# AlexandreRouma/SDRPlusPlus

Hardware: NVIDIA H100
Metric: complex IQ MSamples/s through FFT + 8-VFO WFM chain (higher is better)
Workload: dtype f32

## Files before the change

### sdrplusplus_b200/csrc/api.cpp

```cpp
#include "../../include/b200dsp.h"
#include "engine.h"
#include <chrono>
#include <map>
#include <cmath>
#include <cstdio>
#include <cstring>
#include <cstdlib>
#include <algorithm>

using namespace b200;

static int g_device = -1;

static int ensure_device() {
    int n = 0;
    cudaError_t e = cudaGetDeviceCount(&n);
    if (e != cudaSuccess || n <= 0) {
        set_error("no usable CUDA device (%s): libb200dsp has no CPU fallback", e == cudaSuccess ? "0 devices" : cudaGetErrorString(e));
        cudaGetLastError();
        return B200_ENODEV;
    }
    if (g_device < 0) { g_device = 0; }
    B200_CK(cudaSetDevice(g_device));
    return 0;
// ... 59 lines not shown
    out->mode = pl.mode;
    out->predec_ratio = pl.predec_ratio;
    out->interp = pl.interp;
    out->decim = pl.decim;
    out->ntaps = (int)pl.rtaps.size();
    out->taps_per_phase = pl.taps_per_phase;
    if (pl.use_decim) {
        const DecimPlan* dp = find_decim_plan(pl.predec_ratio);
        if (!dp) { set_error("no decimation plan for ratio %d", pl.predec_ratio); return B200_ENOPLAN; }
        out->nstages = (int)dp->stages.size();
        for (int i = 0; i < out->nstages && i < 8; i++) {
            out->stage_decim[i] = dp->stages[i].decim;
            out->stage_taps[i] = (int)dp->stages[i].taps.size();
        }
    }
    return 0;
}

static int bytes_per_sample(int fmt) { return fmt == B200_FMT_CF32 ? 8 : (fmt == B200_FMT_CS16 ? 4 : 2); }
static int ilog2(int n) { int l = 0; while ((1 << l) < n) { l++; } return l; }

struct FftCore {
    FftPlanDev plan;
    DevBuf tw, twf, win, work;
    int size = 0, nz = 0, window = 0;
    int create(int size_, int nz_, int window_, int max_batch = 1) {
        if (size_ < 8 || size_ > (1 << 22) || (size_ & (size_ - 1))) { set_error("FFT size %d must be a power of two in [8, 4194304]", size_); return B200_EINVAL; }
        if (nz_ < 1 || nz_ > size_) { set_error("bad nz %d", nz_); return B200_EINVAL; }
        size = size_; nz = nz_; window = window_;
        memset(&plan, 0, sizeof(plan));
        plan.N = size; plan.logN = ilog2(size);
        if (size <= 8192) { plan.N1 = size; plan.logN1 = plan.logN; plan.N2 = 1; plan.logN2 = 0; }
        else {
            plan.logN1 = (plan.logN + 1) / 2; plan.N1 = 1 << plan.logN1;
            plan.logN2 = plan.logN - plan.logN1; plan.N2 = 1 << plan.logN2;
        }
        plan.TW = std::max(plan.N1, plan.N2); plan.logTW = ilog2(plan.TW);
        std::vector<float2> t((size_t)plan.TW);
        for (int k = 0; k < plan.TW; k++) {
            double a = -2.0 * 3.14159265358979323846 * (double)k / (double)plan.TW;
            t[k] = make_float2((float)std::cos(a), (float)std::sin(a));
        }
        int rc;
        if ((rc = tw.alloc(t.size() * sizeof(float2)))) { return rc; }
        B200_CK(cudaMemcpy(tw.p, t.data(), t.size() * sizeof(float2), cudaMemcpyHostToDevice));
        std::vector<float> w = fft_window(window, nz);
        if ((rc = win.alloc((size_t)nz * sizeof(float)))) { return rc; }
        B200_CK(cudaMemcpy(win.p, w.data(), (size_t)nz * sizeof(float), cudaMemcpyHostToDevice));
        if ((rc = work.alloc((size_t)size * sizeof(float2) * (size_t)(max_batch > 0 ? max_batch : 1)))) { return rc; }
        plan.tw = tw.as<float2>(); plan.window = win.as<float>(); plan.nz = nz;
        plan.tw_fine = nullptr;
        if (plan.N2 > 1) {
            const int nf = size / plan.TW;
            std::vector<float2> f((size_t)nf);
            for (int j = 0; j < nf; j++) {
                double a = -2.0 * 3.14159265358979323846 * (double)j / (double)size;
                f[j] = make_float2((float)std::cos(a), (float)std::sin(a));
            }
            if ((rc = twf.alloc(f.size() * sizeof(float2)))) { return rc; }
            B200_CK(cudaMemcpy(twf.p, f.data(), f.size() * sizeof(float2), cudaMemcpyHostToDevice));
            plan.tw_fine = twf.as<float2>();
        }
        B200_CK(cudaDeviceSynchronize());
        return 0;
    }
};

static_assert(sizeof(b200_rds_symbol) == 8 && sizeof(RdsSym) == sizeof(b200_rds_symbol), "one RDS symbol record is 8 bytes");
struct RdsCore {
    DevBuf state, taps, bank;
    RdsState init;
    RdsJob proto;
    int create(cudaStream_t s);
    int reset(cudaStream_t s);
    RdsJob job(const float2* in, int n, RdsSym* out, int out_cap, int* count) const {
        RdsJob J = proto;
        J.in = in; J.n = n; J.out = out; J.out_cap = out_cap; J.count = count;
        return J;
    }
};
int RdsCore::create(cudaStream_t s) {
    const std::vector<float> bp = bandpass_c_taps(0.0, 2375.0, 100.0, 5000.0, false);
    const std::vector<float> bk = mm_interp_bank(RDS_MM_PHASES, RDS_MM_TAPS);
    const int nt = (int)bp.size() / 2;
// ... 49 lines not shown

struct b200_fe {
    double fs = 0;
    int max_chunk = 0;
    Scheduler sch;
    cudaStream_t own_stream = nullptr, copy_stream = nullptr, fft_stream = nullptr, tail_stream = nullptr, join_stream = nullptr;
    cudaEvent_t ev_tail_done[FE_SLOTS] = {};
    cudaEvent_t ev_fft_go = nullptr, ev_fft_done = nullptr, ev_lines_free = nullptr;
    bool overlap = true;
    bool lines_busy = false;
    float* lines_override = nullptr;
    bool fft_async = true;
    bool fft_join_pending = false;
    std::vector<std::unique_ptr<VfoSlot>> vfos;
    std::mutex mtx;
    DevBuf in_dev[FE_SLOTS];
    bool fft_on = false;
    FftCore fft;
    double fft_rate = 0;
    int skip = 0;
    DevBuf frame, lines;
    int max_lines = 0;
    unsigned long long pos = 0, fstart = 0;
    cudaEvent_t ev_h2d[FE_SLOTS] = {}, ev_compute[FE_SLOTS] = {}, ev_out[FE_SLOTS] = {};
    bool slot_used[FE_SLOTS] = {};
    int max_inflight = 2;
    unsigned long long nsub = 0, nwait = 0;
    int fft_serial = 0;
    int host_direct = -1;
    long long host_ns[4] = { 0, 0, 0, 0 };
    float scale16 = 1.0f / 32768.0f, scale8 = 1.0f / 128.0f;
    int decim = 1;
    double fs_eff = 0;
    bool dc_block = false, invert_iq = false;
    Chain pre;
    Scheduler sch_pre;
    DevBuf pp[FE_SLOTS];
    DevBuf dc_state, dc_segA, dc_segB;
    int max_eff = 0;
    int* rds_count = nullptr;
    struct RdsPend { int id, n_in, bound; };
    std::vector<RdsPend> rds_pend[FE_SLOTS];
    b200_outputs* rds_out[FE_SLOTS] = {};
};

static float fe_ingest_scale(const b200_fe* fe, int fmt) {
// ... 297 lines not shown
    if (!strcmp(key, "s1_stages")) { kernels_set_xd_tma_stages(value); return 0; }
    if (!strcmp(key, "s1_diag")) { kernels_set_xd_tma_diag(value); return 0; }
    if (!strcmp(key, "s1_ctas")) { kernels_set_xd_tma_ctas(value); return 0; }
    if (!strcmp(key, "tails") || !strncmp(key, "ft_", 3)) {
        if (b200_fe_vfo_count(fe) > 0) { set_error("'%s' must be chosen before VFOs are added", key); return B200_ESTATE; }
        if (!strcmp(key, "tails")) { kernels_set_tail_variant(value >= 1 ? 1 : 0); fe->sch.fuse.on = value >= 2; return 0; }
        if (!strcmp(key, "ft_ob")) { fe->sch.fuse.ob_force = value; return 0; }
        if (!strcmp(key, "ft_obmax")) { fe->sch.fuse.ob_max = value; return 0; }
        if (!strcmp(key, "ft_smem_kb")) { fe->sch.fuse.smem_limit = value * 1024; return 0; }
        if (!strcmp(key, "ft_threads")) { fe->sch.fuse.threads = value; return 0; }
        if (!strcmp(key, "ft_direct")) { fe->sch.fuse.direct = value != 0; return 0; }
        if (!strcmp(key, "ft_prereg")) { fe->sch.fuse.pre_reg = value; return 0; }
        if (!strcmp(key, "ft_regall")) { fe->sch.fuse.reg_all = value != 0; return 0; }
    }
    if (!strcmp(key, "fft")) { kernels_set_fft_variant(value); return 0; }
    if (!strcmp(key, "fft_cta")) { kernels_set_fft_cta(value); return 0; }
    if (!strcmp(key, "host_direct")) { fe->host_direct = value; return 0; }
    if (!strcmp(key, "inflight")) {
        if (value < 1 || value > FE_SLOTS) { set_error("inflight: 1 ... %d", FE_SLOTS); return B200_EINVAL; }
        fe->max_inflight = value;
        return 0;
    }
    if (!strcmp(key, "fft_serial")) { fe->fft_serial = value; return 0; }
    if (!strcmp(key, "graph")) { fe->sch.graph_tails = value; if (value == 0) { fe->sch.drop_graphs(); } return 0; }
    if (!strcmp(key, "graph_max_count")) { fe->sch.graph_max_count = value; return 0; }
    if (!strcmp(key, "pdl")) { kernels_set_pdl(value); fe->sch.drop_graphs(); return 0; }
    if (!strcmp(key, "tail_split")) { fe->sch.tail_split = value; fe->sch.drop_graphs(); return 0; }
    if (!strcmp(key, "time_s1")) { fe->sch.time_s1 = value != 0; for (auto& t : fe->sch.timers) { t.used = 0; } return 0; }
    set_error("unknown option %s", key);
    return B200_EINVAL;
}

extern "C" int b200_fe_s1_stats(b200_fe* fe, double* ms_total, int* launches) {
    if (!fe || !ms_total || !launches) { set_error("null argument"); return B200_EINVAL; }
    return fe->sch.s1_stats(ms_total, launches);
}
extern "C" int b200_fe_group_stats(b200_fe* fe, int group, double* ms_total, int* launches) {
    if (!fe || !ms_total || !launches) { set_error("null argument"); return B200_EINVAL; }
    return fe->sch.group_stats(group, ms_total, launches);
}

extern "C" int b200_fe_reset(b200_fe* fe) {
    if (!fe) { set_error("null fe"); return B200_EINVAL; }
    std::lock_guard<std::mutex> lck(fe->mtx);
    B200_CK(cudaDeviceSynchronize());
    for (auto& v : fe->vfos) {
// ... 49 lines not shown
    const unsigned long long pos = fe->pos, end = pos + (unsigned long long)count;
    const unsigned long long nz = (unsigned long long)fe->fft.nz, interval = nz + (unsigned long long)fe->skip;
    const int bps = bytes_per_sample(fmt);
    const float isc = fe_ingest_scale(fe, fmt);
    fe->fft.plan.in_scale = isc;
    cudaStream_t main_s = fe->sch.stream;
    const bool async = fe->fft_async || fe->sch.tail_stream != nullptr;
    float* const lines_base = fe->lines_override ? fe->lines_override : fe->lines.as<float>();
    cudaStream_t s = async ? fe->fft_stream : main_s;
    bool forked = false;
    cudaEvent_t t_fft = nullptr;
    auto fork = [&]() -> int {
        if (async && !forked) {
            B200_CK(cudaEventRecord(fe->ev_fft_go, main_s));
            B200_CK(cudaStreamWaitEvent(s, fe->ev_fft_go, 0));
            if (fe->lines_busy) { B200_CK(cudaStreamWaitEvent(s, fe->ev_lines_free, 0)); }
            trace_mark("fft start", s);
            t_fft = fe->sch.timer_begin(2, s);
            forked = true;
        }
        return 0;
    };
    int rc = 0;
    if (fe->fstart < pos) {
        const unsigned long long fend = fe->fstart + nz;
        const unsigned long long lo = pos, hi = std::min(fend, end);
        if (hi > lo) {
            if ((rc = fork())) { return rc; }
            cudaError_t e = launch_convert_cf32(dptr, fmt, fe->frame.as<float2>() + (size_t)(lo - fe->fstart), (int)(hi - lo), isc, s);
            if (e != cudaSuccess) { return cuda_fail(e, "launch_convert_cf32"); }
            fe->sch.launches++;
        }
        if (fend <= end) {
            if ((rc = fork())) { return rc; }
            int nl = 0;
            cudaError_t e = launch_fft_frame(fe->fft.plan, fe->frame.p, FMT_CF32, fe->fft.work.as<float2>(), lines_base, nullptr, s, &nl);
            if (e != cudaSuccess) { return cuda_fail(e, "launch_fft_frame"); }
            fe->sch.launches += nl;
            (*nlines)++;
            fe->fstart += interval;
        }
    }
    if (fe->fstart >= pos && fe->fstart + nz <= end) {
        int nb = (int)((end - fe->fstart - nz) / interval) + 1;
        if (*nlines + nb > fe->max_lines) { set_error("FFT line buffer overflow"); return B200_ECAP; }
        if ((rc = fork())) { return rc; }
        const char* src = (const char*)dptr + (size_t)(fe->fstart - pos) * bps;
        int nl = 0;
        cudaError_t e = launch_fft_frames(fe->fft.plan, src, fmt, fe->fft.work.as<float2>(),
                                          lines_base + (size_t)(*nlines) * fe->fft.size, nullptr, s, &nl, nb,
                                          (long long)interval * bps);
        if (e != cudaSuccess) { return cuda_fail(e, "launch_fft_frames"); }
        fe->sch.launches += nl;
        *nlines += nb;
        fe->fstart += interval * (unsigned long long)nb;
    }
    if (fe->fstart < end && fe->fstart >= pos) {
        const unsigned long long lo = fe->fstart, hi = end;
        if (hi > lo) {
            if ((rc = fork())) { return rc; }
            const char* src = (const char*)dptr + (size_t)(lo - pos) * bps;
            cudaError_t e = launch_convert_cf32(src, fmt, fe->frame.as<float2>(), (int)(hi - lo), isc, s);
            if (e != cudaSuccess) { return cuda_fail(e, "launch_convert_cf32"); }
            fe->sch.launches++;
        }
    }
    if (forked) {
        if (t_fft) { B200_CK(cudaEventRecord(t_fft, s)); }
        trace_mark("fft done", s);
        B200_CK(cudaEventRecord(fe->ev_fft_done, s));
        fe->fft_join_pending = true;
        if (fe->fft_serial && s != main_s) { B200_CK(cudaStreamWaitEvent(main_s, fe->ev_fft_done, 0)); }
    }
    fe->pos = end;
    return 0;
}

extern "C" int b200_fe_submit(b200_fe* fe, const void* iq, int count, int in_fmt, int in_mem, b200_outputs* out) {
    if (!fe || !out || (count > 0 && !iq)) { set_error("null argument"); return B200_EINVAL; }
    if (count < 0 || count > fe->max_chunk) { set_error("count %d exceeds max_chunk %d", count, fe->max_chunk); return B200_ECAP; }
    if (in_fmt < 0 || in_fmt > 2) { set_error("bad input format"); return B200_EINVAL; }
    if (fe->nsub - fe->nwait >= (unsigned long long)fe->max_inflight) { set_error("%d chunks already in flight: call b200_fe_wait", fe->max_inflight); return B200_ESTATE; }
    std::lock_guard<std::mutex> lck(fe->mtx);
    const long long hp0 = host_clock_ns();
    apply_pending(fe);
    const int slot = (int)(fe->nsub % FE_SLOTS);
    cudaStream_t s = fe->sch.stream;
// ... 958 lines not shown
```

### sdrplusplus_b200/csrc/fft_reg.cuh

```cuda
#pragma once

__device__ constexpr float FR_COS[16] = { 1.000000000e+00f, 9.807852804e-01f, 9.238795325e-01f, 8.314696123e-01f, 7.071067812e-01f, 5.555702330e-01f,
                                          3.826834324e-01f, 1.950903220e-01f, 0.0f, -1.950903220e-01f, -3.826834324e-01f, -5.555702330e-01f,
                                          -7.071067812e-01f, -8.314696123e-01f, -9.238795325e-01f, -9.807852804e-01f };
__device__ constexpr float FR_SIN[16] = { 0.000000000e+00f, 1.950903220e-01f, 3.826834324e-01f, 5.555702330e-01f, 7.071067812e-01f, 8.314696123e-01f,
                                          9.238795325e-01f, 9.807852804e-01f, 1.0f, 9.807852804e-01f, 9.238795325e-01f, 8.314696123e-01f,
                                          7.071067812e-01f, 5.555702330e-01f, 3.826834324e-01f, 1.950903220e-01f };

template <int R, int K>
__device__ __forceinline__ float2 fr_mul_w(float2 v) {
    constexpr int k32 = K * (32 / R);
    if constexpr (k32 == 0) { return v; }
    else if constexpr (k32 == 8) { return make_float2(v.y, -v.x); }
    else if constexpr (k32 == 4) { return make_float2((v.x + v.y) * RSQRT2, (v.y - v.x) * RSQRT2); }
    else if constexpr (k32 == 12) { return make_float2((v.y - v.x) * RSQRT2, -(v.x + v.y) * RSQRT2); }
    else {
        constexpr float c = FR_COS[k32], s = FR_SIN[k32];
        return make_float2(fmaf(v.y, s, v.x * c), fmaf(-v.x, s, v.y * c));
    }
}
template <int R, int H, int I>
__device__ __forceinline__ void fr_stage(float2 (&a)[R]) {
    constexpr int blk = I / H, j = I % H, i0 = blk * 2 * H + j;
    const float2 u = a[i0], v = a[i0 + H];
    a[i0] = make_float2(u.x + v.x, u.y + v.y);
    a[i0 + H] = fr_mul_w<2 * H, j>(make_float2(u.x - v.x, u.y - v.y));
    if constexpr (I + 1 < R / 2) { fr_stage<R, H, I + 1>(a); }
    else if constexpr (H > 1) { fr_stage<R, H / 2, 0>(a); }
}
template <int R>
__device__ __forceinline__ void fr_dft(float2 (&a)[R]) { fr_stage<R, R / 2, 0>(a); }
template <int R>
__host__ __device__ constexpr int fr_brev(int c) {
    int r = 0;
    for (int bit = 1; bit < R; bit <<= 1) { r = (r << 1) | ((c & bit) ? 1 : 0); }
    return r;
}
template <int RA, int RB> struct FrGeom {
    static constexpr int n = RA * RB;
    static constexpr int TP = RA > RB ? RA : RB;
    static constexpr int crow = RB + 1;
    static constexpr int pitch = ((RA * crow + 13) / 16) * 16 + 2;
};

template <int RA, int RB>
__device__ __forceinline__ void fr_transform(float2 (&v)[RA > RB ? RA : RB], float2* ex, int t, const float2* __restrict__ tw, int twsh) {
    using G = FrGeom<RA, RB>;
    if (t < RB) {
        float2 a[RA];
#pragma unroll
        for (int i = 0; i < RA; i++) { a[i] = v[i]; }
        fr_dft<RA>(a);
#pragma unroll
        for (int c = 0; c < RA; c++) {
            float2 y = a[fr_brev<RA>(c)];
            if (c > 0) { y = cmulf(y, __ldg(tw + ((size_t)(t * c) << twsh))); }
            ex[c * G::crow + t] = y;
        }
    }
    __syncthreads();
    if (t < RA) {
        float2 b[RB];
#pragma unroll
        for (int i = 0; i < RB; i++) { b[i] = ex[t * G::crow + i]; }
        fr_dft<RB>(b);
#pragma unroll
        for (int i = 0; i < RB; i++) { v[i] = b[i]; }
    }
}

template <int FMT, int RA, int RB, int C, int MINB>
__global__ void __launch_bounds__(C * FrGeom<RA, RB>::TP, MINB) k_fftr_p1(const __grid_constant__ FftPlanDev pl, const void* __restrict__ src0,
                                                                    float2* __restrict__ work0, long long src_stride_bytes) {
    using G = FrGeom<RA, RB>;
    extern __shared__ __align__(16) float2 smem[];
    const int N2 = pl.N2;
    const void* src = reinterpret_cast<const char*>(src0) + (size_t)blockIdx.y * src_stride_bytes;
    float2* work = work0 + (size_t)blockIdx.y * pl.N;
    const int col = threadIdx.x % C, t = threadIdx.x / C;
    const int n2 = blockIdx.x * C + col;
    float2 v[G::TP];
    if (t < RB) {
#pragma unroll
        for (int a = 0; a < RA; a++) { v[a] = load_windowed<FMT>(pl, src, (a * RB + t) * N2 + n2); }
    }
    fr_transform<RA, RB>(v, smem + col * G::pitch, t, pl.tw, pl.logTW - pl.logN1);
    if (t < RA) {
        const int s = pl.logN - pl.logTW;
        const unsigned msk = (1u << s) - 1u;
#pragma unroll
        for (int d = 0; d < RB; d++) {
            const int k1 = t + RA * d;
            const unsigned e = (unsigned)k1 * (unsigned)n2;
            const float2 w = cmulf(__ldg(pl.tw + (e >> s)), __ldg(pl.tw_fine + (e & msk)));
            work[(size_t)k1 * N2 + n2] = cmulf(v[fr_brev<RB>(d)], w);
        }
    }
}

template <int RA, int RB, int R>
__global__ void __launch_bounds__(R * FrGeom<RA, RB>::TP) k_fftr_p2(const __grid_constant__ FftPlanDev pl, const float2* __restrict__ work0,
                                                                    float* __restrict__ out_db0) {
    using G = FrGeom<RA, RB>;
    extern __shared__ __align__(16) float2 smem[];
    const int N1 = pl.N1, N2 = pl.N2;
    const float2* work = work0 + (size_t)blockIdx.y * pl.N;
    float* out_db = out_db0 + (size_t)blockIdx.y * pl.N;
    const int t = threadIdx.x % G::TP, row = threadIdx.x / G::TP;
    const int r0 = blockIdx.x * R;
    float2 v[G::TP];
    if (t < RB) {
        const float2* __restrict__ p = work + (size_t)(r0 + row) * N2 + t;
#pragma unroll
        for (int a = 0; a < RA; a++) { v[a] = __ldg(p + a * RB); }
    }
    fr_transform<RA, RB>(v, smem + row * G::pitch, t, pl.tw, pl.logTW - pl.logN2);
    __syncthreads();
    float* T = reinterpret_cast<float*>(smem);
    const float nf = 1.0f / ((float)pl.N * (float)pl.N);
    if (t < RA) {
#pragma unroll
        for (int d = 0; d < RB; d++) { T[(t + RA * d) * (R + 1) + row] = power_db(v[fr_brev<RB>(d)], nf); }
    }
    __syncthreads();
    for (int idx = threadIdx.x; idx < G::n * R; idx += R * G::TP) {
        const int k2 = idx / R, rl = idx - k2 * R;
        out_db[(size_t)(r0 + rl) + (size_t)N1 * k2] = T[k2 * (R + 1) + rl];
    }
}
```

### sdrplusplus_b200/csrc/kernels.cu

```cuda
#include "kernels.cuh"
#include <unordered_map>
#include <mutex>
#include <math.h>
#include <string.h>
#include <algorithm>

template <int FMT>
__device__ __forceinline__ float2 load_iq(const void* __restrict__ p, long long i, float sc) {
    if (FMT == FMT_CF32) {
        return __ldg(reinterpret_cast<const float2*>(p) + i);
    }
    else if (FMT == FMT_CS16) {
        short2 v = __ldg(reinterpret_cast<const short2*>(p) + i);
        return make_float2((float)v.x * sc, (float)v.y * sc);
    }
    else {
        char2 v = __ldg(reinterpret_cast<const char2*>(p) + i);
        return make_float2((float)v.x * sc, (float)v.y * sc);
    }
}

template <int FMT>
__device__ __forceinline__ float2 load_x(const XdParams& p, long long i) {
    if (i >= 0) {
// ... 435 lines not shown
        for (int t = tid; t < per * C; t += nthr) {
            int c, bi;
            if (BATCH_INNER) { c = t & (C - 1); bi = t >> logC; }
            else { bi = t & (per - 1); c = t >> logper; }
            const int base = bi * 2;
            float2 a0 = s[fft_addr<BATCH_INNER>(base + 0, c, C, pitch)];
            float2 a1 = s[fft_addr<BATCH_INNER>(base + 1, c, C, pitch)];
            s[fft_addr<BATCH_INNER>(base + 0, c, C, pitch)] = cadd(a0, a1);
            s[fft_addr<BATCH_INNER>(base + 1, c, C, pitch)] = csub(a0, a1);
        }
        __syncthreads();
    }
}

__device__ __forceinline__ int bitrev(int k, int bits) { return (int)(__brev((unsigned)k) >> (32 - bits)); }

__device__ __forceinline__ float power_db(float2 X, float normFactSq) {
    float m2 = (X.x * X.x + X.y * X.y) * normFactSq;
    float l = log2f(m2);
    if (isinf(l)) { l = copysignf(127.0f, l); }
    return l * 3.01029995663981209120f;
}

template <int FMT>
__device__ __forceinline__ float2 load_windowed(const FftPlanDev& pl, const void* __restrict__ src, int n) {
    if (n >= pl.nz) { return make_float2(0.0f, 0.0f); }
    float2 x = load_iq<FMT>(src, n, pl.in_scale);
    float w = __ldg(pl.window + n);
    return make_float2(x.x * w, x.y * w);
}

template <int FMT>
__global__ void __launch_bounds__(512) k_fft_single(const __grid_constant__ FftPlanDev pl, const void* __restrict__ src0,
                                                      float* __restrict__ out_db0, float2* __restrict__ out_raw,
                                                      long long src_stride_bytes) {
    extern __shared__ __align__(16) float2 smem[];
    const int N = pl.N;
    const void* src = reinterpret_cast<const char*>(src0) + (size_t)blockIdx.y * src_stride_bytes;
    float* out_db = out_db0 + (size_t)blockIdx.y * N;
#pragma unroll 4
    for (int i = threadIdx.x; i < N; i += blockDim.x) { smem[padf(i)] = load_windowed<FMT>(pl, src, i); }
    __syncthreads();
    fft_dif_smem<false>(smem, pl.logN, 1, N, pl.tw, pl.logTW);
    const float nf = 1.0f / ((float)N * (float)N);
    for (int k = threadIdx.x; k < N; k += blockDim.x) {
        float2 X = smem[padf(bitrev(k, pl.logN))];
        out_db[k] = power_db(X, nf);
        if (out_raw) { out_raw[k] = X; }
    }
}

template <int FMT>
__global__ void __launch_bounds__(512) k_fft_p1(const __grid_constant__ FftPlanDev pl, const void* __restrict__ src0,
                                                  float2* __restrict__ work0, int C, long long src_stride_bytes) {
    extern __shared__ __align__(16) float2 smem[];
    const int N1 = pl.N1, N2 = pl.N2;
    const void* src = reinterpret_cast<const char*>(src0) + (size_t)blockIdx.y * src_stride_bytes;
    float2* work = work0 + (size_t)blockIdx.y * pl.N;
    const int c0 = blockIdx.x * C;
#pragma unroll 4
    for (int t = threadIdx.x; t < N1 * C; t += blockDim.x) {
        int n1 = t / C, c = t - n1 * C;
        smem[padf(t)] = load_windowed<FMT>(pl, src, n1 * N2 + c0 + c);
    }
    __syncthreads();
    fft_dif_smem<true>(smem, pl.logN1, C, 0, pl.tw, pl.logTW);
    const float scale = -2.0f / (float)pl.N;
    for (int t = threadIdx.x; t < N1 * C; t += blockDim.x) {
        int k1 = t / C, c = t - k1 * C;
        float2 a = smem[padf(bitrev(k1, pl.logN1) * C + c)];
        int n2 = c0 + c;
        float sn, cs;
        sincospif((float)(k1 * n2) * scale, &sn, &cs);
        work[(size_t)k1 * N2 + n2] = cmulf(a, make_float2(cs, sn));
    }
}

__global__ void __launch_bounds__(512) k_fft_p2(const __grid_constant__ FftPlanDev pl, const float2* __restrict__ work0,
                                                  float* __restrict__ out_db0, float2* __restrict__ out_raw, int R) {
    extern __shared__ __align__(16) float2 smem[];
    const int N1 = pl.N1, N2 = pl.N2;
    const float2* work = work0 + (size_t)blockIdx.y * pl.N;
    float* out_db = out_db0 + (size_t)blockIdx.y * pl.N;
    const int pitch = N2 + 1;
    const int r0 = blockIdx.x * R;
#pragma unroll 4
// ... 536 lines not shown
cudaError_t launch_m2s(const M2SParams& p, cudaStream_t s) {
    if (p.max_n <= 0 || p.njobs <= 0) { return cudaSuccess; }
    dim3 grid(cdiv(p.max_n, 256), p.njobs);
    k_m2s<<<grid, 256, 0, s>>>(p);
    return cudaGetLastError();
}
cudaError_t launch_rxl(const RxlParams& p, cudaStream_t s) {
    if (p.max_n <= 0 || p.njobs <= 0) { return cudaSuccess; }
    dim3 grid(cdiv(p.max_n, 256), p.njobs);
    k_rxl<<<grid, 256, 0, s>>>(p);
    return cudaGetLastError();
}
cudaError_t launch_scale(const ScaleParams& p, cudaStream_t s) {
    if (p.max_n <= 0 || p.njobs <= 0) { return cudaSuccess; }
    dim3 grid(cdiv(p.max_n, 256), p.njobs);
    k_scale<<<grid, 256, 0, s>>>(p);
    return cudaGetLastError();
}
cudaError_t launch_carry(const CarryParams& p, cudaStream_t s) {
    if (p.njobs <= 0) { return cudaSuccess; }
    return launch_chain(k_carry, dim3((unsigned)p.njobs), dim3(256), 0, s, p);
}

template <int FMT>
static cudaError_t launch_fft_fmt(const FftPlanDev& pl, const void* src, float2* work, float* out_db, float2* out_raw,
                                  cudaStream_t s, int* nlaunch, int nbatch, long long src_stride_bytes) {
    cudaError_t e;
    if (pl.N1 == pl.N) {
        size_t smem = ((size_t)pl.N + (pl.N >> 4) + 2) * sizeof(float2);
        e = set_smem(k_fft_single<FMT>, smem);
        if (e != cudaSuccess) { return e; }
        int thr = pl.N / 8 < 32 ? 32 : (pl.N / 8 > 512 ? 512 : pl.N / 8);
        k_fft_single<FMT><<<dim3(1, nbatch), thr, smem, s>>>(pl, src, out_db, out_raw, src_stride_bytes);
        if (nlaunch) { (*nlaunch)++; }
        return cudaGetLastError();
    }
    if (g_fft_variant >= 1 && !out_raw && pl.tw_fine && pl.logN1 >= 8 && pl.logN1 <= 10 && pl.logN2 >= 8 && pl.logN2 <= 10) {
#define FR_P1(RA, RB, CC)                                                                                      \
        do {                                                                                                   \
            const size_t sm = (size_t)CC * FrGeom<RA, RB>::pitch * sizeof(float2);                             \
            e = set_smem(k_fftr_p1<FMT, RA, RB, CC, 2>, sm);                                                   \
            if (e != cudaSuccess) { return e; }                                                                \
            k_fftr_p1<FMT, RA, RB, CC, 2><<<dim3(pl.N2 / CC, nbatch), CC * FrGeom<RA, RB>::TP, sm, s>>>(pl, src, work, src_stride_bytes); \
        } while (0)
#define FR_P2(RA, RB, RR)                                                                                      \
        do {                                                                                                   \
            const size_t sm = (size_t)RR * FrGeom<RA, RB>::pitch * sizeof(float2);                             \
            e = set_smem(k_fftr_p2<RA, RB, RR>, sm);                                                           \
            if (e != cudaSuccess) { return e; }                                                                \
            k_fftr_p2<RA, RB, RR><<<dim3(pl.N1 / RR, nbatch), RR * FrGeom<RA, RB>::TP, sm, s>>>(pl, work, out_db); \
        } while (0)
        if (g_fft_cta == 4) {
            if (pl.logN1 == 10) { FR_P1(32, 32, 4); } else if (pl.logN1 == 9) { FR_P1(16, 32, 4); } else { FR_P1(16, 16, 4); }
        }
        else {
            if (pl.logN1 == 10) { FR_P1(32, 32, 8); } else if (pl.logN1 == 9) { FR_P1(16, 32, 8); } else { FR_P1(16, 16, 8); }
        }
        e = cudaGetLastError();
        if (e != cudaSuccess) { return e; }
        if (g_fft_cta == 4) {
            if (pl.logN2 == 10) { FR_P2(32, 32, 4); } else if (pl.logN2 == 9) { FR_P2(16, 32, 4); } else { FR_P2(16, 16, 4); }
        }
        else {
            if (pl.logN2 == 10) { FR_P2(32, 32, 8); } else if (pl.logN2 == 9) { FR_P2(16, 32, 8); } else { FR_P2(16, 16, 8); }
        }
#undef FR_P1
#undef FR_P2
        if (nlaunch) { (*nlaunch) += 2; }
        return cudaGetLastError();
    }
    int C = 16;
    while (C > 4 && (pl.N2 / C) * nbatch < 2 * num_sms()) { C >>= 1; }
    while ((size_t)pl.N1 * C * sizeof(float2) > 196608 && C > 1) { C >>= 1; }
    if (C > pl.N2) { C = pl.N2; }
    int R = 16;
    while (R > 4 && (pl.N1 / R) * nbatch < 2 * num_sms()) { R >>= 1; }
    while ((size_t)R * (pl.N2 + 1) * sizeof(float2) > 196608 && R > 1) { R >>= 1; }
    if (R > pl.N1) { R = pl.N1; }
    size_t smem1 = ((size_t)pl.N1 * C + ((size_t)pl.N1 * C >> 4) + 2) * sizeof(float2);
    size_t smem2 = ((size_t)R * (pl.N2 + 1) + ((size_t)R * (pl.N2 + 1) >> 4) + 2) * sizeof(float2);
    e = set_smem(k_fft_p1<FMT>, smem1);
    if (e != cudaSuccess) { return e; }
    e = set_smem(k_fft_p2, smem2);
    if (e != cudaSuccess) { return e; }
    const int thr1 = (pl.N1 / 8) * C >= 512 ? 512 : 256, thr2 = (pl.N2 / 8) * R >= 512 ? 512 : 256;
    k_fft_p1<FMT><<<dim3(pl.N2 / C, nbatch), thr1, smem1, s>>>(pl, src, work, C, src_stride_bytes);
    e = cudaGetLastError();
    if (e != cudaSuccess) { return e; }
    k_fft_p2<<<dim3(pl.N1 / R, nbatch), thr2, smem2, s>>>(pl, work, out_db, out_raw, R);
    if (nlaunch) { (*nlaunch) += 2; }
    return cudaGetLastError();
}

cudaError_t launch_fft_frames(const FftPlanDev& pl, const void* src, int fmt, float2* work, float* out_db,
                              float2* out_raw, cudaStream_t s, int* nlaunch, int nbatch, long long src_stride_bytes) {
    if (nbatch <= 0) { return cudaSuccess; }
    if (fmt == FMT_CF32) { return launch_fft_fmt<FMT_CF32>(pl, src, work, out_db, out_raw, s, nlaunch, nbatch, src_stride_bytes); }
    if (fmt == FMT_CS16) { return launch_fft_fmt<FMT_CS16>(pl, src, work, out_db, out_raw, s, nlaunch, nbatch, src_stride_bytes); }
    return launch_fft_fmt<FMT_CS8>(pl, src, work, out_db, out_raw, s, nlaunch, nbatch, src_stride_bytes);
}
cudaError_t launch_fft_frame(const FftPlanDev& pl, const void* src, int fmt, float2* work, float* out_db,
                             float2* out_raw, cudaStream_t s, int* nlaunch) {
    return launch_fft_frames(pl, src, fmt, work, out_db, out_raw, s, nlaunch, 1, 0);
}

cudaError_t launch_convert_cf32(const void* src, int fmt, float2* dst, int n, float scale, cudaStream_t s) {
    if (n <= 0) { return cudaSuccess; }
    int grid = cdiv(n, 256);
    if (fmt == FMT_CF32) { k_convert<FMT_CF32><<<grid, 256, 0, s>>>(src, dst, n, scale); }
    else if (fmt == FMT_CS16) { k_convert<FMT_CS16><<<grid, 256, 0, s>>>(src, dst, n, scale); }
    else { k_convert<FMT_CS8><<<grid, 256, 0, s>>>(src, dst, n, scale); }
    return cudaGetLastError();
}

__global__ void __launch_bounds__(256) k_export(const float* __restrict__ in, long long n, int type, float scalar, void* __restrict__ out) {
    const long long i = (long long)blockIdx.x * blockDim.x + threadIdx.x;
    if (i >= n) { return; }
    const float x = __ldg(in + i);
    if (type == EXP_U8) {
        const float v = __fadd_rn(__fmul_rn(x, 127.0f), 128.0f);
        reinterpret_cast<unsigned char*>(out)[i] = (unsigned char)__float2int_rz(v);
    }
    else if (type == EXP_I8) {
        float r = __fmul_rn(x, scalar);
        r = fminf(fmaxf(r, -128.0f), 127.0f);
        reinterpret_cast<signed char*>(out)[i] = (signed char)__float2int_rn(r);
// ... 56 lines not shown
```

### sdrplusplus_b200/csrc/kernels.cuh

```cuda
#pragma once
#include <cuda_runtime.h>
#include <stdint.h>

#define B200_BATCH 16

enum { FMT_CF32 = 0, FMT_CS16 = 1, FMT_CS8 = 2 };

struct XdJob {
    float2* out;
    const float2* gpad;
    unsigned long long phase0;
    unsigned long long w;
    int offset;
    int n_out;
    int T;
    const float* h;
    unsigned long long w_prev;
    int retuned;
};
struct XdParams {
    const void* in;
    const float2* hist;
    int hist_len;
    int count;
// ... 235 lines not shown
    int esize;
    int bfmt;
    float scale;
};
#define CARRY_BATCH 64
struct CarryParams { int njobs; CarryJob job[CARRY_BATCH]; };

struct ChanParams {
    const float2* in;
    float2* u;
    const float* h;
    int M, P, n_out;
};
cudaError_t launch_channelizer(const ChanParams& p, float2* y, const float2* tw, cudaStream_t s, int* nlaunch);

struct FftPlanDev {
    int N, logN;
    int N1, logN1;
    int N2, logN2;
    const float2* tw;
    int TW, logTW;
    const float2* tw_fine;
    const float* window;
    float in_scale;
    int nz;
};

cudaError_t launch_xlate_decim(const XdParams& p, int fmt, int variant, cudaStream_t s, int* nlaunch);
cudaError_t launch_xd_edge(const XdParams& p, int fmt, cudaStream_t s, int* nlaunch);
cudaError_t launch_fir_c(const FirParams& p, cudaStream_t s);
cudaError_t launch_fir_reg(const FirParams& p, cudaStream_t s);
cudaError_t launch_firr_reg(const FirRParams& p, cudaStream_t s);
cudaError_t launch_poly(const PolyParams& p, cudaStream_t s);
cudaError_t launch_quad(const QuadParams& p, cudaStream_t s);
cudaError_t launch_fir_r(const FirRParams& p, cudaStream_t s);
cudaError_t launch_seq(const SeqParams& p, cudaStream_t s);
cudaError_t launch_m2s(const M2SParams& p, cudaStream_t s);
cudaError_t launch_scale(const ScaleParams& p, cudaStream_t s);
cudaError_t launch_carry(const CarryParams& p, cudaStream_t s);
cudaError_t launch_fft_frame(const FftPlanDev& pl, const void* src, int fmt, float2* work, float* out_db,
                             float2* out_raw, cudaStream_t s, int* nlaunch);
cudaError_t launch_fft_frames(const FftPlanDev& pl, const void* src, int fmt, float2* work, float* out_db,
                              float2* out_raw, cudaStream_t s, int* nlaunch, int nbatch, long long src_stride_bytes);
struct DcbParams {
    const void* in;
    float2* out;
    int fmt;
    int count;
    float in_scale;
    float rate;
    int dc_on, conj_on;
    float2* state;
    float2* segB;
    float* segA;
    int nseg;
};
cudaError_t launch_preproc(const DcbParams& p, cudaStream_t s, int* nlaunch);
cudaError_t launch_convert_cf32(const void* src, int fmt, float2* dst, int n, float scale, cudaStream_t s);
enum { EXP_U8 = 0, EXP_I8 = 1, EXP_I16 = 2, EXP_I32 = 3 };
cudaError_t launch_export(const float* in, long long n, int type, float scalar, void* out, cudaStream_t s);
cudaError_t launch_index_max(const float* in, long long n, float* out_val, cudaStream_t s);
cudaError_t launch_zoom_hold_tbl(const float* line, const int* start, const int* len, int out_size, float* out,
                                 float* hold, float hold_speed, cudaStream_t s);
int kernels_max_smem_optin();
void kernels_set_tail_variant(int v);
void kernels_set_fft_variant(int v);
// ... 7 lines not shown
```

Baseline: 94590.

## Stage FFT twiddles in shared memory, pre-permute window, fuse frame carry-over

The register-based two-pass FFT kernels can now copy the twiddle tables into shared memory and read a window array pre-permuted per thread for vectorised float4 loads. The frame that straddles two chunks is now read directly from a raw-format carry buffer plus the new chunk, so it no longer needs a separate convert or serial single-frame launch. This removes global twiddle gathers and extra kernel launches, at the cost of more shared memory per block, a register cap, and more complicated frame bookkeeping.

New measurement: 101,300 (median of 6 runs). +7.1%, better.

```diff
diff --git a/sdrplusplus_b200/csrc/api.cpp b/sdrplusplus_b200/csrc/api.cpp
--- a/sdrplusplus_b200/csrc/api.cpp
+++ b/sdrplusplus_b200/csrc/api.cpp
@@ -105,7 +105,7 @@
 
 struct FftCore {
     FftPlanDev plan;
-    DevBuf tw, twf, win, work;
+    DevBuf tw, twf, win, winp, work;
     int size = 0, nz = 0, window = 0;
     int create(int size_, int nz_, int window_, int max_batch = 1) {
         if (size_ < 8 || size_ > (1 << 22) || (size_ & (size_ - 1))) { set_error("FFT size %d must be a power of two in [8, 4194304]", size_); return B200_EINVAL; }
@@ -143,6 +143,22 @@
             if ((rc = twf.alloc(f.size() * sizeof(float2)))) { return rc; }
             B200_CK(cudaMemcpy(twf.p, f.data(), f.size() * sizeof(float2), cudaMemcpyHostToDevice));
             plan.tw_fine = twf.as<float2>();
+        }
+        plan.window_p = nullptr;
+        if (fft_plan_uses_reg(plan)) {
+            const int RA = plan.logN1 == 8 ? 16 : (plan.logN1 == 9 ? 16 : 32), RB = plan.logN1 == 8 ? 16 : 32;
+            std::vector<float> wp((size_t)size, 0.0f);
+            for (int n2 = 0; n2 < plan.N2; n2++) {
+                for (int t = 0; t < RB; t++) {
+                    for (int a = 0; a < RA; a++) {
+                        const long long n = (long long)(a * RB + t) * plan.N2 + n2;
+                        if (n < nz) { wp[((size_t)n2 * RB + t) * RA + a] = w[(size_t)n]; }
+                    }
+                }
+            }
+            if ((rc = winp.alloc(wp.size() * sizeof(float)))) { return rc; }
+            B200_CK(cudaMemcpy(winp.p, wp.data(), wp.size() * sizeof(float), cudaMemcpyHostToDevice));
+            plan.window_p = winp.as<float>();
         }
         B200_CK(cudaDeviceSynchronize());
         return 0;
@@ -238,6 +254,9 @@
     DevBuf frame, lines;
     int max_lines = 0;
     unsigned long long pos = 0, fstart = 0;
+    int frame_fmt = FMT_CF32;
+    float frame_scale = 0.0f;
+    int fft_v = 1;
     cudaEvent_t ev_h2d[FE_SLOTS] = {}, ev_compute[FE_SLOTS] = {}, ev_out[FE_SLOTS] = {};
     bool slot_used[FE_SLOTS] = {};
     int max_inflight = 2;
@@ -581,6 +600,12 @@
         return 0;
     }
     if (!strcmp(key, "fft_serial")) { fe->fft_serial = value; return 0; }
+    if (!strcmp(key, "fft_v")) {
+        if (value != 0 && value != 1) { set_error("fft_v: 0 or 1"); return B200_EINVAL; }
+        std::lock_guard<std::mutex> lck(fe->mtx);
+        fe->fft_v = value;
+        return 0;
+    }
     if (!strcmp(key, "graph")) { fe->sch.graph_tails = value; if (value == 0) { fe->sch.drop_graphs(); } return 0; }
     if (!strcmp(key, "graph_max_count")) { fe->sch.graph_max_count = value; return 0; }
     if (!strcmp(key, "pdl")) { kernels_set_pdl(value); fe->sch.drop_graphs(); return 0; }
@@ -676,7 +701,20 @@
         return 0;
     };
     int rc = 0;
-    if (fe->fstart < pos) {
+    char* const frame = (char*)fe->frame.p;
+    const bool pending = fe->fstart < pos;
+    const bool same_fmt = fe->frame_fmt == fmt && (fmt == FMT_CF32 || fe->frame_scale == isc);
+    if (pending && (!fe->fft_v || !same_fmt) && fe->frame_fmt != FMT_CF32) {
+        if ((rc = fork())) { return rc; }
+        const int len = (int)(pos - fe->fstart);
+        cudaError_t e = launch_convert_cf32(frame, fe->frame_fmt, fe->fft.work.as<float2>(), len, fe->frame_scale, s);
+        if (e != cudaSuccess) { return cuda_fail(e, "launch_convert_cf32"); }
+        fe->sch.launches++;
+        B200_CK(cudaMemcpyAsync(frame, fe->fft.work.p, (size_t)len * sizeof(float2), cudaMemcpyDeviceToDevice, s));
+        fe->frame_fmt = FMT_CF32;
+        fe->frame_scale = 0.0f;
+    }
+    if (pending && (!fe->fft_v || !same_fmt)) {
         const unsigned long long fend = fe->fstart + nz;
         const unsigned long long lo = pos, hi = std::min(fend, end);
         if (hi > lo) {
@@ -688,22 +726,29 @@
         if (fend <= end) {
             if ((rc = fork())) { return rc; }
             int nl = 0;
-            cudaError_t e = launch_fft_frame(fe->fft.plan, fe->frame.p, FMT_CF32, fe->fft.work.as<float2>(), lines_base, nullptr, s, &nl);
-            if (e != cudaSuccess) { return cuda_fail(e, "launch_fft_frame"); }
+            const FftFrames fr{ fe->frame.p, nullptr, 0, 0, 1 };
+            cudaError_t e = launch_fft_frames(fe->fft.plan, fr, FMT_CF32, fe->fft.work.as<float2>(), lines_base, nullptr, s, &nl, fe->fft_v != 0);
+            if (e != cudaSuccess) { return cuda_fail(e, "launch_fft_frames"); }
             fe->sch.launches += nl;
             (*nlines)++;
             fe->fstart += interval;
         }
     }
-    if (fe->fstart >= pos && fe->fstart + nz <= end) {
+    else if (pending && fe->fstart + nz > end) {
+        if (count > 0) {
+            if ((rc = fork())) { return rc; }
+            B200_CK(cudaMemcpyAsync(frame + (size_t)(pos - fe->fstart) * bps, dptr, (size_t)count * bps, cudaMemcpyDeviceToDevice, s));
+        }
+    }
+    const unsigned long long split = fe->fstart < pos ? pos - fe->fstart : 0;
+    if (fe->fstart + nz <= end) {
         int nb = (int)((end - fe->fstart - nz) / interval) + 1;
         if (*nlines + nb > fe->max_lines) { set_error("FFT line buffer overflow"); return B200_ECAP; }
         if ((rc = fork())) { return rc; }
-        const char* src = (const char*)dptr + (size_t)(fe->fstart - pos) * bps;
+        const FftFrames fr{ (const char*)dptr + (size_t)(fe->fstart + split - pos) * bps, frame, (long long)interval, (int)split, nb };
         int nl = 0;
-        cudaError_t e = launch_fft_frames(fe->fft.plan, src, fmt, fe->fft.work.as<float2>(),
-                                          lines_base + (size_t)(*nlines) * fe->fft.size, nullptr, s, &nl, nb,
-                                          (long long)interval * bps);
+        cudaError_t e = launch_fft_frames(fe->fft.plan, fr, fmt, fe->fft.work.as<float2>(), lines_base + (size_t)(*nlines) * fe->fft.size,
+                                          nullptr, s, &nl, fe->fft_v != 0);
         if (e != cudaSuccess) { return cuda_fail(e, "launch_fft_frames"); }
         fe->sch.launches += nl;
         *nlines += nb;
@@ -711,12 +756,19 @@
     }
     if (fe->fstart < end && fe->fstart >= pos) {
         const unsigned long long lo = fe->fstart, hi = end;
-        if (hi > lo) {
-            if ((rc = fork())) { return rc; }
-            const char* src = (const char*)dptr + (size_t)(lo - pos) * bps;
+        if ((rc = fork())) { return rc; }
+        const char* src = (const char*)dptr + (size_t)(lo - pos) * bps;
+        if (fe->fft_v) {
+            B200_CK(cudaMemcpyAsync(frame, src, (size_t)(hi - lo) * bps, cudaMemcpyDeviceToDevice, s));
+            fe->frame_fmt = fmt;
+            fe->frame_scale = isc;
+        }
+        else {
             cudaError_t e = launch_convert_cf32(src, fmt, fe->frame.as<float2>(), (int)(hi - lo), isc, s);
             if (e != cudaSuccess) { return cuda_fail(e, "launch_convert_cf32"); }
             fe->sch.launches++;
+            fe->frame_fmt = FMT_CF32;
+            fe->frame_scale = 0.0f;
         }
     }
     if (forked) {
diff --git a/sdrplusplus_b200/csrc/fft_reg.cuh b/sdrplusplus_b200/csrc/fft_reg.cuh
--- a/sdrplusplus_b200/csrc/fft_reg.cuh
+++ b/sdrplusplus_b200/csrc/fft_reg.cuh
@@ -43,7 +43,7 @@
     static constexpr int pitch = ((RA * crow + 13) / 16) * 16 + 2;
 };
 
-template <int RA, int RB>
+template <int RA, int RB, bool TAB>
 __device__ __forceinline__ void fr_transform(float2 (&v)[RA > RB ? RA : RB], float2* ex, int t, const float2* __restrict__ tw, int twsh) {
     using G = FrGeom<RA, RB>;
     if (t < RB) {
@@ -54,7 +54,7 @@
 #pragma unroll
         for (int c = 0; c < RA; c++) {
             float2 y = a[fr_brev<RA>(c)];
-            if (c > 0) { y = cmulf(y, __ldg(tw + ((size_t)(t * c) << twsh))); }
+            if (c > 0) { y = cmulf(y, TAB ? tw[(t * c) << twsh] : __ldg(tw + ((size_t)(t * c) << twsh))); }
             ex[c * G::crow + t] = y;
         }
     }
@@ -69,22 +69,49 @@
     }
 }
 
-template <int FMT, int RA, int RB, int C, int MINB>
-__global__ void __launch_bounds__(C * FrGeom<RA, RB>::TP, MINB) k_fftr_p1(const __grid_constant__ FftPlanDev pl, const void* __restrict__ src0,
-                                                                    float2* __restrict__ work0, long long src_stride_bytes) {
+__device__ __forceinline__ void fr_stage_table(float2* dst, const float2* __restrict__ src, int n) {
+    for (int i = threadIdx.x; i < n / 2; i += blockDim.x) {
+        reinterpret_cast<float4*>(dst)[i] = __ldg(reinterpret_cast<const float4*>(src) + i);
+    }
+}
+template <int RA, int RB>
+__host__ __device__ constexpr size_t fr_smem_tiles(int X) { return (size_t)X * FrGeom<RA, RB>::pitch; }
+
+template <int FMT, int RA, int RB, int C, bool TAB>
+__global__ void __launch_bounds__(C * FrGeom<RA, RB>::TP) __maxnreg__(TAB ? 144 : (C == 8 ? 128 : 255)) k_fftr_p1(const __grid_constant__ FftPlanDev pl, const __grid_constant__ FftFrames fr,
+                                                                    float2* __restrict__ work0) {
     using G = FrGeom<RA, RB>;
     extern __shared__ __align__(16) float2 smem[];
     const int N2 = pl.N2;
-    const void* src = reinterpret_cast<const char*>(src0) + (size_t)blockIdx.y * src_stride_bytes;
-    float2* work = work0 + (size_t)blockIdx.y * pl.N;
+    const int f = blockIdx.y;
+    float2* work = work0 + (size_t)f * pl.N;
     const int col = threadIdx.x % C, t = threadIdx.x / C;
     const int n2 = blockIdx.x * C + col;
+    float2* const tws = smem + fr_smem_tiles<RA, RB>(C);
+    float2* const fine = tws + pl.TW;
+    if (TAB) {
+        fr_stage_table(tws, pl.tw, pl.TW);
+        fr_stage_table(fine, pl.tw_fine, pl.N >> pl.logTW);
+    }
     float2 v[G::TP];
     if (t < RB) {
+        const FrameSrc fs = frame_src<FMT>(fr, f);
 #pragma unroll
-        for (int a = 0; a < RA; a++) { v[a] = load_windowed<FMT>(pl, src, (a * RB + t) * N2 + n2); }
+        for (int a = 0; a < RA; a++) { v[a] = load_frame<FMT>(pl, fs, (a * RB + t) * N2 + n2, !TAB); }
+        if (TAB) {
+            const float4* __restrict__ wp = reinterpret_cast<const float4*>(pl.window_p + ((size_t)n2 * RB + t) * RA);
+#pragma unroll
+            for (int q = 0; q < RA / 4; q++) {
+                const float4 w = __ldg(wp + q);
+                v[4 * q + 0] = make_float2(v[4 * q + 0].x * w.x, v[4 * q + 0].y * w.x);
+                v[4 * q + 1] = make_float2(v[4 * q + 1].x * w.y, v[4 * q + 1].y * w.y);
+                v[4 * q + 2] = make_float2(v[4 * q + 2].x * w.z, v[4 * q + 2].y * w.z);
+                v[4 * q + 3] = make_float2(v[4 * q + 3].x * w.w, v[4 * q + 3].y * w.w);
+            }
+        }
     }
-    fr_transform<RA, RB>(v, smem + col * G::pitch, t, pl.tw, pl.logTW - pl.logN1);
+    if (TAB) { __syncthreads(); }
+    fr_transform<RA, RB, TAB>(v, smem + col * G::pitch, t, TAB ? tws : pl.tw, pl.logTW - pl.logN1);
     if (t < RA) {
         const int s = pl.logN - pl.logTW;
         const unsigned msk = (1u << s) - 1u;
@@ -92,13 +119,13 @@
         for (int d = 0; d < RB; d++) {
             const int k1 = t + RA * d;
             const unsigned e = (unsigned)k1 * (unsigned)n2;
-            const float2 w = cmulf(__ldg(pl.tw + (e >> s)), __ldg(pl.tw_fine + (e & msk)));
+            const float2 w = TAB ? cmulf(tws[e >> s], fine[e & msk]) : cmulf(__ldg(pl.tw + (e >> s)), __ldg(pl.tw_fine + (e & msk)));
             work[(size_t)k1 * N2 + n2] = cmulf(v[fr_brev<RB>(d)], w);
         }
     }
 }
 
-template <int RA, int RB, int R>
+template <int RA, int RB, int R, bool TAB>
 __global__ void __launch_bounds__(R * FrGeom<RA, RB>::TP) k_fftr_p2(const __grid_constant__ FftPlanDev pl, const float2* __restrict__ work0,
                                                                     float* __restrict__ out_db0) {
     using G = FrGeom<RA, RB>;
@@ -108,13 +135,16 @@
     float* out_db = out_db0 + (size_t)blockIdx.y * pl.N;
     const int t = threadIdx.x % G::TP, row = threadIdx.x / G::TP;
     const int r0 = blockIdx.x * R;
+    float2* const tws = smem + fr_smem_tiles<RA, RB>(R);
+    if (TAB) { fr_stage_table(tws, pl.tw, pl.TW); }
     float2 v[G::TP];
     if (t < RB) {
         const float2* __restrict__ p = work + (size_t)(r0 + row) * N2 + t;
 #pragma unroll
         for (int a = 0; a < RA; a++) { v[a] = __ldg(p + a * RB); }
     }
-    fr_transform<RA, RB>(v, smem + row * G::pitch, t, pl.tw, pl.logTW - pl.logN2);
+    if (TAB) { __syncthreads(); }
+    fr_transform<RA, RB, TAB>(v, smem + row * G::pitch, t, TAB ? tws : pl.tw, pl.logTW - pl.logN2);
     __syncthreads();
     float* T = reinterpret_cast<float*>(smem);
     const float nf = 1.0f / ((float)pl.N * (float)pl.N);
diff --git a/sdrplusplus_b200/csrc/kernels.cu b/sdrplusplus_b200/csrc/kernels.cu
--- a/sdrplusplus_b200/csrc/kernels.cu
+++ b/sdrplusplus_b200/csrc/kernels.cu
@@ -481,24 +481,31 @@
     return l * 3.01029995663981209120f;
 }
 
+struct FrameSrc { const char* lo; const char* hi; int lim; };
 template <int FMT>
-__device__ __forceinline__ float2 load_windowed(const FftPlanDev& pl, const void* __restrict__ src, int n) {
+__device__ __forceinline__ FrameSrc frame_src(const FftFrames& fr, int f) {
+    constexpr int bps = FMT == FMT_CF32 ? 8 : (FMT == FMT_CS16 ? 4 : 2);
+    return { reinterpret_cast<const char*>(fr.pre), reinterpret_cast<const char*>(fr.chunk) + ((long long)f * fr.stride - fr.split) * bps,
+             f == 0 ? fr.split : 0 };
+}
+template <int FMT>
+__device__ __forceinline__ float2 load_frame(const FftPlanDev& pl, const FrameSrc& fs, int n, bool windowed) {
     if (n >= pl.nz) { return make_float2(0.0f, 0.0f); }
-    float2 x = load_iq<FMT>(src, n, pl.in_scale);
-    float w = __ldg(pl.window + n);
+    const float2 x = load_iq<FMT>(n < fs.lim ? fs.lo : fs.hi, n, pl.in_scale);
+    if (!windowed) { return x; }
+    const float w = __ldg(pl.window + n);
     return make_float2(x.x * w, x.y * w);
 }
 
 template <int FMT>
-__global__ void __launch_bounds__(512) k_fft_single(const __grid_constant__ FftPlanDev pl, const void* __restrict__ src0,
-                                                      float* __restrict__ out_db0, float2* __restrict__ out_raw,
-                                                      long long src_stride_bytes) {
+__global__ void __launch_bounds__(512) k_fft_single(const __grid_constant__ FftPlanDev pl, const __grid_constant__ FftFrames fr,
+                                                      float* __restrict__ out_db0, float2* __restrict__ out_raw) {
     extern __shared__ __align__(16) float2 smem[];
     const int N = pl.N;
-    const void* src = reinterpret_cast<const char*>(src0) + (size_t)blockIdx.y * src_stride_bytes;
     float* out_db = out_db0 + (size_t)blockIdx.y * N;
+    const FrameSrc fs = frame_src<FMT>(fr, blockIdx.y);
 #pragma unroll 4
-    for (int i = threadIdx.x; i < N; i += blockDim.x) { smem[padf(i)] = load_windowed<FMT>(pl, src, i); }
+    for (int i = threadIdx.x; i < N; i += blockDim.x) { smem[padf(i)] = load_frame<FMT>(pl, fs, i, true); }
     __syncthreads();
     fft_dif_smem<false>(smem, pl.logN, 1, N, pl.tw, pl.logTW);
     const float nf = 1.0f / ((float)N * (float)N);
@@ -510,17 +517,17 @@
 }
 
 template <int FMT>
-__global__ void __launch_bounds__(512) k_fft_p1(const __grid_constant__ FftPlanDev pl, const void* __restrict__ src0,
-                                                  float2* __restrict__ work0, int C, long long src_stride_bytes) {
+__global__ void __launch_bounds__(512) k_fft_p1(const __grid_constant__ FftPlanDev pl, const __grid_constant__ FftFrames fr,
+                                                  float2* __restrict__ work0, int C) {
     extern __shared__ __align__(16) float2 smem[];
     const int N1 = pl.N1, N2 = pl.N2;
-    const void* src = reinterpret_cast<const char*>(src0) + (size_t)blockIdx.y * src_stride_bytes;
     float2* work = work0 + (size_t)blockIdx.y * pl.N;
     const int c0 = blockIdx.x * C;
+    const FrameSrc fs = frame_src<FMT>(fr, blockIdx.y);
 #pragma unroll 4
     for (int t = threadIdx.x; t < N1 * C; t += blockDim.x) {
         int n1 = t / C, c = t - n1 * C;
-        smem[padf(t)] = load_windowed<FMT>(pl, src, n1 * N2 + c0 + c);
+        smem[padf(t)] = load_frame<FMT>(pl, fs, n1 * N2 + c0 + c, true);
     }
     __syncthreads();
     fft_dif_smem<true>(smem, pl.logN1, C, 0, pl.tw, pl.logTW);
@@ -1103,33 +1110,52 @@
     return launch_chain(k_carry, dim3((unsigned)p.njobs), dim3(256), 0, s, p);
 }
 
+bool fft_plan_uses_reg(const FftPlanDev& pl) {
+    return pl.N2 > 1 && pl.logN1 >= 8 && pl.logN1 <= 10 && pl.logN2 >= 8 && pl.logN2 <= 10;
+}
+
 template <int FMT>
-static cudaError_t launch_fft_fmt(const FftPlanDev& pl, const void* src, float2* work, float* out_db, float2* out_raw,
-                                  cudaStream_t s, int* nlaunch, int nbatch, long long src_stride_bytes) {
+static cudaError_t launch_fft_fmt(const FftPlanDev& pl, const FftFrames& fr, float2* work, float* out_db, float2* out_raw,
+                                  cudaStream_t s, int* nlaunch, bool tables) {
     cudaError_t e;
+    const int nbatch = fr.nbatch;
     if (pl.N1 == pl.N) {
         size_t smem = ((size_t)pl.N + (pl.N >> 4) + 2) * sizeof(float2);
         e = set_smem(k_fft_single<FMT>, smem);
         if (e != cudaSuccess) { return e; }
         int thr = pl.N / 8 < 32 ? 32 : (pl.N / 8 > 512 ? 512 : pl.N / 8);
-        k_fft_single<FMT><<<dim3(1, nbatch), thr, smem, s>>>(pl, src, out_db, out_raw, src_stride_bytes);
+        k_fft_single<FMT><<<dim3(1, nbatch), thr, smem, s>>>(pl, fr, out_db, out_raw);
         if (nlaunch) { (*nlaunch)++; }
         return cudaGetLastError();
     }
-    if (g_fft_variant >= 1 && !out_raw && pl.tw_fine && pl.logN1 >= 8 && pl.logN1 <= 10 && pl.logN2 >= 8 && pl.logN2 <= 10) {
+    if (g_fft_variant >= 1 && !out_raw && pl.tw_fine && pl.window_p && fft_plan_uses_reg(pl)) {
 #define FR_P1(RA, RB, CC)                                                                                      \
         do {                                                                                                   \
-            const size_t sm = (size_t)CC * FrGeom<RA, RB>::pitch * sizeof(float2);                             \
-            e = set_smem(k_fftr_p1<FMT, RA, RB, CC, 2>, sm);                                                   \
-            if (e != cudaSuccess) { return e; }                                                                \
-            k_fftr_p1<FMT, RA, RB, CC, 2><<<dim3(pl.N2 / CC, nbatch), CC * FrGeom<RA, RB>::TP, sm, s>>>(pl, src, work, src_stride_bytes); \
+            const size_t sm = (fr_smem_tiles<RA, RB>(CC) + (tables ? (size_t)pl.TW + (pl.N >> pl.logTW) : 0)) * sizeof(float2); \
+            if (tables) {                                                                                      \
+                e = set_smem(k_fftr_p1<FMT, RA, RB, CC, true>, sm);                                         \
+                if (e != cudaSuccess) { return e; }                                                            \
+                k_fftr_p1<FMT, RA, RB, CC, true><<<dim3(pl.N2 / CC, nbatch), CC * FrGeom<RA, RB>::TP, sm, s>>>(pl, fr, work); \
+            }                                                                                                  \
+            else {                                                                                             \
+                e = set_smem(k_fftr_p1<FMT, RA, RB, CC, false>, sm);                                        \
+                if (e != cudaSuccess) { return e; }                                                            \
+                k_fftr_p1<FMT, RA, RB, CC, false><<<dim3(pl.N2 / CC, nbatch), CC * FrGeom<RA, RB>::TP, sm, s>>>(pl, fr, work); \
+            }                                                                                                  \
         } while (0)
 #define FR_P2(RA, RB, RR)                                                                                      \
         do {                                                                                                   \
-            const size_t sm = (size_t)RR * FrGeom<RA, RB>::pitch * sizeof(float2);                             \
-            e = set_smem(k_fftr_p2<RA, RB, RR>, sm);                                                           \
-            if (e != cudaSuccess) { return e; }                                                                \
-            k_fftr_p2<RA, RB, RR><<<dim3(pl.N1 / RR, nbatch), RR * FrGeom<RA, RB>::TP, sm, s>>>(pl, work, out_db); \
+            const size_t sm = (fr_smem_tiles<RA, RB>(RR) + (tables ? (size_t)pl.TW : 0)) * sizeof(float2);     \
+            if (tables) {                                                                                      \
+                e = set_smem(k_fftr_p2<RA, RB, RR, true>, sm);                                                 \
+                if (e != cudaSuccess) { return e; }                                                            \
+                k_fftr_p2<RA, RB, RR, true><<<dim3(pl.N1 / RR, nbatch), RR * FrGeom<RA, RB>::TP, sm, s>>>(pl, work, out_db); \
+            }                                                                                                  \
+            else {                                                                                             \
+                e = set_smem(k_fftr_p2<RA, RB, RR, false>, sm);                                                \
+                if (e != cudaSuccess) { return e; }                                                            \
+                k_fftr_p2<RA, RB, RR, false><<<dim3(pl.N1 / RR, nbatch), RR * FrGeom<RA, RB>::TP, sm, s>>>(pl, work, out_db); \
+            }                                                                                                  \
         } while (0)
         if (g_fft_cta == 4) {
             if (pl.logN1 == 10) { FR_P1(32, 32, 4); } else if (pl.logN1 == 9) { FR_P1(16, 32, 4); } else { FR_P1(16, 16, 4); }
@@ -1165,7 +1191,7 @@
     e = set_smem(k_fft_p2, smem2);
     if (e != cudaSuccess) { return e; }
     const int thr1 = (pl.N1 / 8) * C >= 512 ? 512 : 256, thr2 = (pl.N2 / 8) * R >= 512 ? 512 : 256;
-    k_fft_p1<FMT><<<dim3(pl.N2 / C, nbatch), thr1, smem1, s>>>(pl, src, work, C, src_stride_bytes);
+    k_fft_p1<FMT><<<dim3(pl.N2 / C, nbatch), thr1, smem1, s>>>(pl, fr, work, C);
     e = cudaGetLastError();
     if (e != cudaSuccess) { return e; }
     k_fft_p2<<<dim3(pl.N1 / R, nbatch), thr2, smem2, s>>>(pl, work, out_db, out_raw, R);
@@ -1173,16 +1199,17 @@
     return cudaGetLastError();
 }
 
-cudaError_t launch_fft_frames(const FftPlanDev& pl, const void* src, int fmt, float2* work, float* out_db,
-                              float2* out_raw, cudaStream_t s, int* nlaunch, int nbatch, long long src_stride_bytes) {
-    if (nbatch <= 0) { return cudaSuccess; }
-    if (fmt == FMT_CF32) { return launch_fft_fmt<FMT_CF32>(pl, src, work, out_db, out_raw, s, nlaunch, nbatch, src_stride_bytes); }
-    if (fmt == FMT_CS16) { return launch_fft_fmt<FMT_CS16>(pl, src, work, out_db, out_raw, s, nlaunch, nbatch, src_stride_bytes); }
-    return launch_fft_fmt<FMT_CS8>(pl, src, work, out_db, out_raw, s, nlaunch, nbatch, src_stride_bytes);
+cudaError_t launch_fft_frames(const FftPlanDev& pl, const FftFrames& fr, int fmt, float2* work, float* out_db,
+                              float2* out_raw, cudaStream_t s, int* nlaunch, bool tables) {
+    if (fr.nbatch <= 0) { return cudaSuccess; }
+    if (fmt == FMT_CF32) { return launch_fft_fmt<FMT_CF32>(pl, fr, work, out_db, out_raw, s, nlaunch, tables); }
+    if (fmt == FMT_CS16) { return launch_fft_fmt<FMT_CS16>(pl, fr, work, out_db, out_raw, s, nlaunch, tables); }
+    return launch_fft_fmt<FMT_CS8>(pl, fr, work, out_db, out_raw, s, nlaunch, tables);
 }
 cudaError_t launch_fft_frame(const FftPlanDev& pl, const void* src, int fmt, float2* work, float* out_db,
                              float2* out_raw, cudaStream_t s, int* nlaunch) {
-    return launch_fft_frames(pl, src, fmt, work, out_db, out_raw, s, nlaunch, 1, 0);
+    const FftFrames fr{ src, nullptr, 0, 0, 1 };
+    return launch_fft_frames(pl, fr, fmt, work, out_db, out_raw, s, nlaunch, true);
 }
 
 cudaError_t launch_convert_cf32(const void* src, int fmt, float2* dst, int n, float scale, cudaStream_t s) {
diff --git a/sdrplusplus_b200/csrc/kernels.cuh b/sdrplusplus_b200/csrc/kernels.cuh
--- a/sdrplusplus_b200/csrc/kernels.cuh
+++ b/sdrplusplus_b200/csrc/kernels.cuh
@@ -281,6 +281,7 @@
     int TW, logTW;
     const float2* tw_fine;
     const float* window;
+    const float* window_p;
     float in_scale;
     int nz;
 };
@@ -297,10 +298,18 @@
 cudaError_t launch_m2s(const M2SParams& p, cudaStream_t s);
 cudaError_t launch_scale(const ScaleParams& p, cudaStream_t s);
 cudaError_t launch_carry(const CarryParams& p, cudaStream_t s);
+struct FftFrames {
+    const void* chunk;
+    const void* pre;
+    long long stride;
+    int split;
+    int nbatch;
+};
 cudaError_t launch_fft_frame(const FftPlanDev& pl, const void* src, int fmt, float2* work, float* out_db,
                              float2* out_raw, cudaStream_t s, int* nlaunch);
-cudaError_t launch_fft_frames(const FftPlanDev& pl, const void* src, int fmt, float2* work, float* out_db,
-                              float2* out_raw, cudaStream_t s, int* nlaunch, int nbatch, long long src_stride_bytes);
+cudaError_t launch_fft_frames(const FftPlanDev& pl, const FftFrames& fr, int fmt, float2* work, float* out_db,
+                              float2* out_raw, cudaStream_t s, int* nlaunch, bool tables);
+bool fft_plan_uses_reg(const FftPlanDev& pl);
 struct DcbParams {
     const void* in;
     float2* out;
```
